# lqhl/rabitq-rs

Hardware: AMD Instinct MI355X
Metric: queries/sec at recall@10>=0.95, GIST-1M d=960, batch=1024 (higher is better)
Workload: dtype u8

## Files before the change

rabitq-rs_amd/csrc/device/k_query.hip:

```cpp
#include <hip/hip_runtime.h>

#include <algorithm>
#include <cstdlib>

#include "launch.hpp"
#include "query_kernels.hpp"
#include "rank_mfma.hpp"
#include "latency.hpp"

namespace rbq {

namespace {
uint32_t next_pow2(uint32_t x) { uint32_t p = 1; while (p < x) p <<= 1; return p; }
}

hipError_t launch_prep(const PrepParams& p, int device, hipStream_t s) {
    if (p.rotator == 0  || p.wg_prep) {
        static LdsAttrCache attr;
        const size_t lds = (size_t)p.D * 4 * 2;
        if (probe_stage(0, reinterpret_cast<const void*>(&k_prep), dim3(p.nq), kThreads, lds)) return hipSuccess;
        hipError_t e = attr.ensure(reinterpret_cast<const void*>(&k_prep), lds, device);
        if (e != hipSuccess) return e;
        hipLaunchKernelGGL(k_prep, dim3(p.nq), dim3(kThreads), lds, s, p.queries, p.dim, p.D, p.Dc, p.rotator, p.rot_blob, p.trunc,
                           p.fac, p.ex_bits, p.rot, p.lut, p.consts, p.rot_hi, p.rot_lo);
// ... 76 lines not shown
    const uint32_t np2 = next_pow2(p.nprobe);
    const size_t lds = (key_window ? 0 : (size_t)np2 * 8) + (size_t)p.D * 4 + kThreads * 4;
    static LdsAttrCache attr, attr_unf;
    const bool unf = p.numeric_variant == (uint32_t)kVarPortable;
    const void* fn = unf ? reinterpret_cast<const void*>(&k_select<true>) : reinterpret_cast<const void*>(&k_select<false>);
    if (probe_stage(2, fn, dim3(p.nq), kThreads, lds)) return hipSuccess;
    hipError_t e = (unf ? attr_unf : attr).ensure(fn, lds, device);
    if (e != hipSuccess) return e;
    if (unf) hipLaunchKernelGGL(k_select<true>, dim3(p.nq), dim3(kThreads), lds, s, (const float*)p.scores, p.nlist, p.nprobe, np2, p.metric, p.rot,
                                p.cent, p.D, p.list_gb0, p.list_n, p.probe, p.wl, p.wl_stride, p.nstream, p.nvec, p.prof_total, p.consts,
                                p.bsum, key_window);
    else hipLaunchKernelGGL(k_select<false>, dim3(p.nq), dim3(kThreads), lds, s, (const float*)p.scores, p.nlist, p.nprobe, np2, p.metric, p.rot,
                       p.cent, p.D, p.list_gb0, p.list_n, p.probe, p.wl, p.wl_stride, p.nstream, p.nvec, p.prof_total, p.consts,
                       p.bsum, key_window);
    return hipGetLastError();
}

namespace {
template <int RM, int V>
hipError_t launch_select_rmv(const SelectParams& p, const SelectGeom& g, size_t lds, int device, hipStream_t s) {
    static LdsAttrCache attr;
    if (probe_stage(2, reinterpret_cast<const void*>(&k_select_mfma<RM, V>), dim3(p.nq), kThreads, lds)) return hipSuccess;
    hipError_t e = attr.ensure(reinterpret_cast<const void*>(&k_select_mfma<RM, V>), lds, device);
    if (e != hipSuccess) return e;
    hipLaunchKernelGGL((k_select_mfma<RM, V>), dim3(p.nq), dim3(kThreads), lds, s, p, g);
    return hipGetLastError();
}
template <int RM>
hipError_t launch_select_rm(const SelectParams& p, const SelectGeom& g, size_t lds, int device, hipStream_t s) {
    if (p.numeric_variant == (uint32_t)kVarAvx2) return launch_select_rmv<RM, kVarAvx2>(p, g, lds, device, s);
    if (p.numeric_variant == (uint32_t)kVarPortable) return launch_select_rmv<RM, kVarPortable>(p, g, lds, device, s);
    return launch_select_rmv<RM, kVarAvx512>(p, g, lds, device, s);
}
}

template <int RM>
size_t select_static_lds() {
    static const size_t v = [] {
        hipFuncAttributes fa;
        if (hipFuncGetAttributes(&fa, reinterpret_cast<const void*>(&k_select_mfma<RM>)) != hipSuccess) { (void)hipGetLastError(); return (size_t)8192; }
        return (size_t)fa.sharedSizeBytes;
    }();
    return v;
}

hipError_t launch_select_mfma(const SelectParams& p, int device, hipStream_t s) {
    SelectGeom g;
    g.cap2 = next_pow2(2 * p.nprobe) < 64u ? 64u : next_pow2(2 * p.nprobe);
    const size_t lds0 = (size_t)g.cap2 * 8 + (size_t)p.D * 4 + kThreads * 4;
    g.row_in_lds = (p.nlist > 4096 && (size_t)p.nlist * 4 <= 65536 &&
                    lds0 + (size_t)p.nlist * 4 + select_static_lds<1>() <= kLdsPerWorkgroupMax) ? 1 : 0;
    size_t lds = lds0 + (g.row_in_lds ? (size_t)p.nlist * 4 : 0);
    g.stage = lds + (size_t)p.nprobe * 16 <= 48 * 1024 ? 1 : 0;
    if (g.stage) lds += (size_t)p.nprobe * 16;
#ifndef RBQ_SEL_ROWS
#define RBQ_SEL_ROWS 4
#endif
    const size_t rowsN = RBQ_SEL_ROWS * ((size_t)p.D + 8) * 4 + 16;
    g.stage_rows = (p.lazy && lds + rowsN <= 64 * 1024) ? (uint32_t)RBQ_SEL_ROWS : 0u;
    g.hx_nv = 0;
    size_t regionN = g.stage_rows ? rowsN : 0;
    if (p.lazy && p.head_exact && p.lut && p.top_k <= kHxMaxVec && p.D % 16 == 0) {
#ifndef RBQ_HX_BUDGET
#define RBQ_HX_BUDGET (16384u * 8u)
#endif
        uint32_t nv = (uint32_t)(((uint32_t)RBQ_HX_BUDGET / p.Dc) / 32u * 32u);
        nv = nv < 64u ? 64u : (nv > kHxMaxVec ? kHxMaxVec : nv);
        const size_t hxN = (hx_scratch_bytes(p.D, p.Dc, p.ex_bits, nv) + 15) & ~(size_t)15;
        if (lds + std::max(regionN, hxN) <= 64 * 1024) { g.hx_nv = nv; regionN = std::max(regionN, hxN); }
    }
    lds += regionN;
    g.cand_cap = (uint32_t)(((g.stage ? (size_t)p.nprobe * 16 : 0) + (g.stage_rows ? rowsN - 16 : 0)) / 8);
    if (p.nlist <= 4096) return launch_select_rm<2>(p, g, lds, device, s);
    if (g.row_in_lds) return launch_select_rm<1>(p, g, lds, device, s);
    return launch_select_rm<0>(p, g, lds, device, s);
}

hipError_t launch_probes_given(const ProbesGivenParams& p, hipStream_t s) {
    if (p.numeric_variant == (uint32_t)kVarPortable)
        hipLaunchKernelGGL(k_probes_given<true>, dim3(p.nq), dim3(kThreads), (size_t)p.D * 4 + kThreads * 4, s, p.list_ids, p.list_counts,
                           p.max_lists, p.nlist, p.metric, p.rot, p.cent, p.D, p.list_gb0, p.list_n, p.probe, p.wl, p.wl_stride, p.nstream,
                           p.consts, p.bsum);
    else hipLaunchKernelGGL(k_probes_given<false>, dim3(p.nq), dim3(kThreads), (size_t)p.D * 4 + kThreads * 4, s, p.list_ids, p.list_counts,
                            p.max_lists, p.nlist, p.metric, p.rot, p.cent, p.D, p.list_gb0, p.list_n, p.probe, p.wl, p.wl_stride, p.nstream,
                            p.consts, p.bsum);
    return hipGetLastError();
}

}
```

rabitq-rs_amd/csrc/device/rank_mfma.hpp:

```cpp
#pragma once
#include "kernels.hpp"

namespace rbq {

#ifndef RBQ_CANON_UNROLL
#define RBQ_CANON_UNROLL 4
#endif
typedef float f32x16 __attribute__((ext_vector_type(16)));

template <int METRIC, int TW>
__global__ __launch_bounds__(256) void k_rank_mfma(const float* __restrict__ rot, const float* __restrict__ cent,
                                                   const QueryConsts* __restrict__ consts,
                                                   const float* __restrict__ cnorm2, uint32_t nq, uint32_t nlist,
                                                   uint32_t D, float* __restrict__ scores) {
    constexpr int BM = 64 * TW, BN = 64 * TW, BK = 32, LD = BK + 1;
    __shared__ float As[BM][LD];
    __shared__ float Bs[BN][LD];
    const uint32_t tid = threadIdx.x, lane = tid & 63u, w = tid >> 6, wm = w >> 1, wn = w & 1u;
    const uint32_t q0 = blockIdx.y * BM, c0 = blockIdx.x * BN;
    f32x16 acc[TW][TW];
#pragma unroll
    for (int a = 0; a < TW; ++a)
#pragma unroll
        for (int b = 0; b < TW; ++b)
// ... 237 lines not shown
    }
    for (uint32_t i = Dmain; i < D; ++i) {
        float p;
        if (METRIC == 0) {
            const float d = qrot[i] - c[i];
            p = d * d;
        } else {
            p = qrot[i] * c[i];
        }
        sum = sum + p;
    }
    return sum;
}

__device__ __forceinline__ void canon_pair2_ip_l2(const float* qrot, const float* __restrict__ c, uint32_t D, uint32_t h,
                                                  float& dot, float& l2) {
    const uint32_t Dmain = D & ~7u;
    float a[4] = {0, 0, 0, 0}, b[4] = {0, 0, 0, 0};
#pragma unroll 4
    for (uint32_t i = 4 * h; i < Dmain; i += 8) {
        const float4 cv = *reinterpret_cast<const float4*>(c + i);
        const float4 qv = *reinterpret_cast<const float4*>(qrot + i);
        const float q4[4] = {qv.x, qv.y, qv.z, qv.w}, c4[4] = {cv.x, cv.y, cv.z, cv.w};
#pragma unroll
        for (int k = 0; k < 4; ++k) {
            const float p = q4[k] * c4[k];
            const float d = q4[k] - c4[k];
            const float r = d * d;
            a[k] = a[k] + p;
            b[k] = b[k] + r;
        }
    }
    float s0 = 0.0f, s1 = 0.0f;
    if (Dmain) {
        s0 = -0.0f; s1 = -0.0f;
#pragma unroll
        for (int l = 0; l < 2; ++l)
#pragma unroll
            for (int k = 0; k < 4; ++k) {
                s0 = s0 + __shfl(a[k], l, 2);
                s1 = s1 + __shfl(b[k], l, 2);
            }
    }
    for (uint32_t i = Dmain; i < D; ++i) {
        const float p = qrot[i] * c[i];
        const float d = qrot[i] - c[i];
        const float r = d * d;
        s0 = s0 + p;
        s1 = s1 + r;
    }
    dot = s0; l2 = s1;
}

#ifdef RBQ_SEL_WAVES
#define RBQ_SEL_BOUNDS __launch_bounds__(kThreads, RBQ_SEL_WAVES)
#else
#define RBQ_SEL_BOUNDS __launch_bounds__(kThreads)
#endif

struct SelectGeom {
    uint32_t cap2;
    int row_in_lds;
    int stage;
    uint32_t stage_rows;
    uint32_t cand_cap;
    uint32_t hx_nv;
};
#ifndef RBQ_HX_TRIGGER
#define RBQ_HX_TRIGGER 6
#endif
#ifndef RBQ_HX_REFINE_MULT
#define RBQ_HX_REFINE_MULT 2
#endif
constexpr uint32_t kHxTrigger = RBQ_HX_TRIGGER;
constexpr uint32_t kHxMaxVec = 256;

template <typename IdxFn>
__device__ __forceinline__ void canon_score_pairs(uint64_t* keys, const float* qrot, const float* __restrict__ cent, uint32_t D, int metric,
                                                  float* grow, uint32_t m, uint32_t tid, IdxFn idx_of) {
    const uint32_t l2 = tid & 1u, grp = tid >> 1;
    for (uint32_t i0 = 0; i0 < m; i0 += kThreads / 2) {
        const uint32_t j = i0 + grp;
        uint32_t cid = 0, e = 0;
        float s = 0.0f;
        if (j < m) {
            e = idx_of(j);
            cid = (uint32_t)keys[e];
            const float* c = cent + (size_t)cid * D;
            if (metric == 0) s = canon_pair2<0>(qrot, c, D, l2);
            else {
                float dl2;
                canon_pair2_ip_l2(qrot, c, D, l2, s, dl2);
                if (l2 == 0) grow[cid] = dl2;
            }
        }
        if (j < m && l2 == 0) keys[e] = make_key(s, cid, metric);
    }
}
template <typename IdxFn>
__device__ __forceinline__ void canon_score_staged(uint64_t* keys, const float* qrot, const float* __restrict__ cent, uint32_t D, int metric,
                                                   float* grow, uint32_t m, uint32_t tid, float* rows, uint32_t RB, IdxFn idx_of) {
    const uint32_t Dp = D + 8u, Dmain = D & ~7u, nv4 = D >> 2;
    for (uint32_t base = 0; base < m; base += RB) {
        const uint32_t nr = m - base < RB ? m - base : RB;
        for (uint32_t x0 = tid; x0 < nr * nv4; x0 += 4 * kThreads) {
            float4 t4[4];
#pragma unroll
            for (int u = 0; u < 4; ++u) {
                const uint32_t x = x0 + (uint32_t)u * kThreads;
                t4[u] = make_float4(0.0f, 0.0f, 0.0f, 0.0f);
                if (x < nr * nv4) {
                    const uint32_t r = x / nv4, j4 = x - r * nv4;
                    const uint32_t cid = (uint32_t)keys[idx_of(base + r)];
                    t4[u] = *reinterpret_cast<const float4*>(cent + (size_t)cid * D + 4 * j4);
                }
            }
#pragma unroll
            for (int u = 0; u < 4; ++u) {
                const uint32_t x = x0 + (uint32_t)u * kThreads;
                if (x < nr * nv4) {
                    const uint32_t r = x / nv4, j4 = x - r * nv4;
                    *reinterpret_cast<float4*>(rows + (size_t)r * Dp + 4 * j4) = t4[u];
                }
            }
        }
// ... 134 lines not shown
        }
    }
}

__device__ __forceinline__ void sort_keys(uint64_t* keys, uint32_t n, uint32_t cap2, uint32_t tid) {
    if (n <= 2 * kThreads) {
        uint64_t my[2] = {~0ull, ~0ull};
        uint32_t rk[2] = {0, 0};
#pragma unroll
        for (int u = 0; u < 2; ++u) if (tid + u * kThreads < n) my[u] = keys[tid + u * kThreads];
        const uint32_t wbase = tid & ~63u;
        if (n > (uint32_t)kThreads) {
#pragma unroll 8
            for (uint32_t j = 0; j < n; ++j) {
                const uint64_t kj = keys[j];
                rk[0] += kj < my[0] ? 1u : 0u;
                rk[1] += kj < my[1] ? 1u : 0u;
            }
        } else if (wbase < n) {
            const uint4* k2 = reinterpret_cast<const uint4*>(keys);
            const uint32_t np2 = (n + 1) >> 1;
#pragma unroll 8
            for (uint32_t j = 0; j < np2; ++j) {
                const uint4 kk = k2[j];
                const uint64_t ka = ((uint64_t)kk.y << 32) | kk.x, kb = ((uint64_t)kk.w << 32) | kk.z;
                rk[0] += (ka < my[0] ? 1u : 0u) + (kb < my[0] ? 1u : 0u);
            }
        }
        __syncthreads();
#pragma unroll
        for (int u = 0; u < 2; ++u) if (tid + u * kThreads < n) keys[rk[u]] = my[u];
        __syncthreads();
    } else {
        for (uint32_t k = 2; k <= cap2; k <<= 1)
            for (uint32_t j = k >> 1; j > 0; j >>= 1) {
                for (uint32_t i = tid; i < cap2; i += kThreads) {
                    const uint32_t ixj = i ^ j;
                    if (ixj > i) {
                        const uint64_t a = keys[i], b = keys[ixj];
                        const bool up = (i & k) == 0;
                        if ((a > b) == up) { keys[i] = b; keys[ixj] = a; }
                    }
                }
                __syncthreads();
            }
    }
}


#ifndef RBQ_HX_EX_ALL
#define RBQ_HX_EX_ALL 0
#endif
#ifndef RBQ_HX_GRANULES
#define RBQ_HX_GRANULES 4
#endif
__host__ __device__ inline size_t hx_scratch_bytes(uint32_t D, uint32_t Dc, uint32_t ex_bits, uint32_t nv) {
    return (size_t)Dc * 4 + (ex_bits ? (size_t)ex_qlen(D, ex_bits) * 4 : 0) + (size_t)nv * 16 + 16;
}
__device__ __forceinline__ uint32_t hx_look8(uint32_t x, const uint8_t* p) {
    uint32_t s = p[x & 15u];
    s += p[16 + ((x >> 4) & 15u)];
    s += p[32 + ((x >> 8) & 15u)];
    s += p[48 + ((x >> 12) & 15u)];
    s += p[64 + ((x >> 16) & 15u)];
    s += p[80 + ((x >> 20) & 15u)];
    s += p[96 + ((x >> 24) & 15u)];
    s += p[112 + (x >> 28)];
    return s;
}
__device__ __forceinline__ bool hx_tame(float x) { return fabsf(x) < 1e30f; }
template <int V, class CostOf>
__device__ __forceinline__ float head_exact_bound(const SelectParams& P, const SelectGeom& G, const QueryConsts& qc, const uint64_t* keys,
                                                  const uint32_t* s_head, const uint32_t* s_hgb, const uint32_t* s_hn, const float* s_hcn,
                                                  uint32_t h, float eps, unsigned char* scratch, const float* qrot, uint32_t* part, uint32_t* hist,
                                                  uint32_t q, uint32_t tid, CostOf&& cost_of) {
    const uint32_t D = P.D, Dc = P.Dc, ex_bits = P.ex_bits, top_k = P.top_k;
    uint32_t r0 = 0, kbest = 0xffffffffu;
    for (uint32_t r = 0; r < h; ++r) {
        const uint32_t k32 = (uint32_t)(keys[s_head[r]] >> 32);
        if (k32 < kbest) { kbest = k32; r0 = r; }
    }
    const float ci = cost_of(kbest);
    const float g_add = ci + 1.01f * eps;
    float ge_lo, ge_hi;
    if (P.metric == 0) { ge_lo = sqrtf(fmaxf(ci - 1.01f * eps, 0.0f)); ge_hi = sqrtf(fmaxf(g_add, 0.0f)); }
    else { const float da = qc.qnorm2 + s_hcn[r0] + 2.0f * ci; ge_lo = sqrtf(fmaxf(da - 4.0f * eps, 0.0f)); ge_hi = sqrtf(fmaxf(da + 4.0f * eps, 0.0f)); }
    const uint32_t gb = s_hgb[r0], nvec = s_hn[r0];
    const uint32_t nv = nvec < G.hx_nv ? nvec : G.hx_nv;
    if (nv < top_k || top_k == 0 || !hx_tame(g_add) || !hx_tame(ge_hi)) return INFINITY;
    if (r0 >= h || (uint64_t)gb + ((nv + 31u) >> 5) > (uint64_t)P.n_blocks) {
        if (tid == 0 && P.fallback_count) atomicAdd(P.fallback_count + 2, 1u);
        return INFINITY;
    }
    if (tid == 0 && P.fallback_count) atomicAdd(P.fallback_count + 3, 1u);
    uint8_t* lutL = scratch;
    float* sq = reinterpret_cast<float*>(scratch + (size_t)Dc * 4);
    const uint32_t qlen = ex_bits ? ex_qlen(D, ex_bits) : 0u;
    float* vEst = sq + qlen;
    float* vLb = vEst + nv;
    float* vIp = vLb + nv;
    float* vU = vIp + nv;
    {
        const uint4* src = reinterpret_cast<const uint4*>(P.lut + (size_t)q * Dc * 4);
        uint4* dst = reinterpret_cast<uint4*>(lutL);
        for (uint32_t i = tid; i < Dc / 4; i += kThreads) dst[i] = src[i];
        for (uint32_t i = tid; i < qlen; i += kThreads) sq[i] = i < D ? qrot[i] : 0.0f;
    }
// ... 96 lines not shown
                const float d = a + m;
                const bool ok = vEst[v] < INFINITY && hx_tame(fa) && hx_tame(fr) && hx_tame(t0) && hx_tame(sacc) && hx_tame(t1) && hx_tame(tt2) &&
                                hx_tame(a) && hx_tame(m) && hx_tame(d);
                vU[j] = ok ? fmaxf(d, vLb[v]) : INFINITY;
            }
        }
    }
    __syncthreads();
    if (tid < R) {
        const float my = vU[tid];
        uint32_t rk = 0;
        for (uint32_t j = 0; j < R; ++j) { const float o = vU[j]; rk += (o < my || (o == my && j < tid)) ? 1u : 0u; }
        if (rk == top_k - 1u) res[0] = my;
    }
    __syncthreads();
    const float r = res[0];
    __syncthreads();
    return r;
}

constexpr uint32_t kSelHead = 4;
constexpr uint32_t kSelTodoMax = 512;
constexpr uint32_t kSelKeptMax = 256;
constexpr uint32_t kSelZoneMax = 1024;

template <int RM, int V = kVarAvx512>
__global__ RBQ_SEL_BOUNDS void k_select_mfma(const SelectParams P, const SelectGeom G) {
    extern __shared__ __align__(16) unsigned char smraw[];
    const uint32_t nlist = P.nlist, nprobe = P.nprobe, cap2 = G.cap2, D = P.D;
    const int metric = P.metric;
    uint64_t* keys = reinterpret_cast<uint64_t*>(smraw);
    float* qrot = reinterpret_cast<float*>(smraw + (size_t)cap2 * 8);
    uint32_t* part = reinterpret_cast<uint32_t*>(qrot + D);
    __shared__ uint32_t hist[256];
    __shared__ uint32_t s_k, s_cnt, s_bad;
    __shared__ unsigned long long s_nvec;
#ifdef RBQ_SEL_STAMPS
    unsigned long long ts[8]; int tn = 0;
#define SSTAMP() ts[tn++] = __builtin_amdgcn_s_memtime()
#else
#define SSTAMP()
#endif
#if defined(RBQ_SEL_STAMPS) && RBQ_SEL_STAMPS == 4
    unsigned long long ls[8] = {0, 0, 0, 0, 0, 0, 0, 0};
#define LSTAMP(i) ls[i] = __builtin_amdgcn_s_memtime()
#else
#define LSTAMP(i)
#endif
    SSTAMP();
    const uint32_t q = blockIdx.x, tid = threadIdx.x;
    float* grow = P.scores + (size_t)q * nlist;
    float* lrow = reinterpret_cast<float*>(part + kThreads);
    uint32_t* pgeo = reinterpret_cast<uint32_t*>(lrow + (RM == 1 ? nlist : 0u));
    float* rows = reinterpret_cast<float*>(smraw + ((reinterpret_cast<unsigned char*>(pgeo + (G.stage ? 4u * nprobe : 0u)) - smraw + 15) & ~(size_t)15));
    constexpr int KPT = 16;
    uint32_t kreg[KPT];
    bool bad_load = false;
    uint64_t* cand = reinterpret_cast<uint64_t*>(pgeo);
    bool use_cand = false;
    uint32_t n_cand = 0;
    auto okey = [&](float s) -> uint32_t {
        int32_t k = total_key(s);
        if (metric == 1) k = ~k;
        return (uint32_t)k ^ 0x80000000u;
    };
    auto cost_of = [&](uint32_t k32) -> float {
        int32_t k = (int32_t)(k32 ^ 0x80000000u);
        if (metric == 1) k = ~k;
        const float s = key_to_float(k);
        return metric == 0 ? s : -s;
    };
    if (RM == 2) {
#pragma unroll
        for (int v = 0; v < KPT / 4; ++v) {
            const uint32_t i = v * 1024u + tid * 4u;
            float4 x = make_float4(0, 0, 0, 0);
            if (i + 3 < nlist) x = *reinterpret_cast<const float4*>(grow + i);
            else { if (i < nlist) x.x = grow[i]; if (i + 1 < nlist) x.y = grow[i + 1]; if (i + 2 < nlist) x.z = grow[i + 2]; }
            bad_load |= !finite_f(x.x) || !finite_f(x.y) || !finite_f(x.z) || !finite_f(x.w);
            kreg[4 * v] = okey(x.x); kreg[4 * v + 1] = okey(x.y); kreg[4 * v + 2] = okey(x.z); kreg[4 * v + 3] = okey(x.w);
        }
    } else if (RM == 1) {
        for (uint32_t i = tid; i < nlist; i += kThreads) lrow[i] = grow[i];
    }
    auto each_key = [&](auto&& body) {
        if (RM == 2) {
#pragma unroll
            for (int u = 0; u < KPT; ++u) {
                const uint32_t i = (uint32_t)(u >> 2) * 1024u + tid * 4u + (uint32_t)(u & 3);
                if (i < nlist) body(i, kreg[u]);
            }
        } else if (RM == 1) {
            for (uint32_t i = tid; i < nlist; i += kThreads) { const float v = lrow[i]; bad_load |= !finite_f(v); body(i, okey(v)); }
        } else if (use_cand) {
            for (uint32_t j = tid; j < n_cand; j += kThreads) { const uint64_t kc = cand[j]; body((uint32_t)kc, (uint32_t)(kc >> 32)); }
        } else {
            for (uint32_t i = tid; i < nlist; i += kThreads) { const float v = grow[i]; bad_load |= !finite_f(v); body(i, okey(v)); }
        }
    };

    {
        float qv[4];
        for (uint32_t i0 = tid; i0 < D; i0 += 4 * kThreads) {
#pragma unroll
            for (int u = 0; u < 4; ++u) qv[u] = i0 + (uint32_t)u * kThreads < D ? P.rot[(size_t)q * D + i0 + (uint32_t)u * kThreads] : 0.0f;
#pragma unroll
            for (int u = 0; u < 4; ++u) if (i0 + (uint32_t)u * kThreads < D) qrot[i0 + (uint32_t)u * kThreads] = qv[u];
        }
    }
    if (tid == 0) { s_k = nprobe - 1; s_cnt = 0; s_nvec = 0; s_bad = 0; }
    __syncthreads();

    SSTAMP();
    bool all = nprobe >= nlist;
    __shared__ uint32_t s_lo, s_hi, s_bin, s_cum, s_h, s_ng, s_w4[4], s_nc;
    auto kth_key = [&](auto&& each, uint32_t k) -> uint32_t {
        if (tid == 0) { s_lo = 0xffffffffu; s_hi = 0u; s_ng = 0u; }
        __syncthreads();
        {
            uint32_t kmn = 0xffffffffu, kmx = 0u;
            each([&](uint32_t, uint32_t key) {
                kmn = key < kmn ? key : kmn;
                kmx = key > kmx ? key : kmx;
            });
            const bool bad = bad_load;
            kmn = wave_min_u32(kmn);
            kmx = ~wave_min_u32(~kmx);
            if ((tid & 63u) == 0) { atomicMin(&s_lo, kmn); atomicMax(&s_hi, kmx); }
            if (bad) s_bad = 1;
        }
        __syncthreads();
        uint32_t lo = s_lo, hi = s_hi;
        while (true) {
            const uint32_t span = hi - lo;
            const uint32_t sh = span < 256u ? 0u : (32u - (uint32_t)__builtin_clz(span)) - 8u;
            hist[tid] = 0;
            __syncthreads();
            each([&](uint32_t, uint32_t key) {
                if (key - lo <= hi - lo) atomicAdd(&hist[(key - lo) >> sh], 1u);
            });
            __syncthreads();
            const uint32_t h = hist[tid];
            uint32_t total;
            const uint32_t excl = block_scan_excl256(h, s_w4, tid, total);
            if (excl <= k && k < excl + h) { s_bin = tid; s_cum = excl; s_h = h; }
            __syncthreads();
            k -= s_cum;
            lo += s_bin << sh;
            const uint32_t width = (sh ? (1u << sh) : 1u) - 1u;
            if (hi - lo > width) hi = lo + width;
            if (sh == 0) break;
            const uint32_t nc = s_h;
            if (nc <= (uint32_t)kThreads) {
                uint32_t* cnd = hist;
                each([&](uint32_t, uint32_t key) {
                    if (key - lo <= hi - lo) cnd[atomicAdd(&s_ng, 1u)] = key;
                });
                __syncthreads();
                if (tid < nc) {
                    const uint32_t my = cnd[tid];
                    uint32_t less = 0, eq = 0;
#pragma unroll 8
                    for (uint32_t j = 0; j < nc; ++j) {
                        const uint32_t kj = cnd[j];
                        less += kj < my ? 1u : 0u;
                        eq += kj == my ? 1u : 0u;
                    }
                    if (less <= k && k < less + eq) s_lo = my;
                }
                __syncthreads();
                lo = s_lo;
                break;
            }
        }
        __syncthreads();
        return lo;
    };
    const QueryConsts qc = P.consts[q];
    const float eps = ((6.0f * (float)D + 16.0f) * 5.9604645e-8f + 4.0f * 1.52587890625e-5f) * (qc.qnorm2 + P.cnorm2_max) * 1.001f;
    auto widen = [&](uint32_t key) -> uint32_t {
        int32_t k = (int32_t)(key ^ 0x80000000u);
        if (metric == 1) k = ~k;
        const float sc = key_to_float(k);
        const float lim = metric == 0 ? sc + 2.0f * eps : sc - 2.0f * eps;
        return finite_f(lim) ? okey(lim) : 0xffffffffu;
    };
    constexpr int KL = 8;
    if (RM == 0 && !all && G.cand_cap >= 4u * nprobe && 2u * nprobe <= (uint32_t)(kThreads * KL)) {
        uint32_t lk[KL];
#pragma unroll
        for (int u = 0; u < KL; ++u) lk[u] = 0xffffffffu;
        constexpr int KU = 8;
        for (uint32_t i0 = tid; i0 < nlist; i0 += kThreads * KU) {
            float vv[KU];
#pragma unroll
            for (int w = 0; w < KU; ++w) { const uint32_t i = i0 + (uint32_t)w * kThreads; vv[w] = i < nlist ? grow[i] : 0.0f; }
#pragma unroll
            for (int w = 0; w < KU; ++w) {
                if (i0 + (uint32_t)w * kThreads < nlist) {
                    const float v = vv[w];
                    bad_load |= !finite_f(v);
                    const uint32_t key = okey(v);
                    if (key < lk[KL - 1]) {
                        lk[KL - 1] = key;
#pragma unroll
                        for (int u = KL - 1; u > 0; --u) {
                            const uint32_t a = lk[u - 1], b = lk[u];
                            lk[u - 1] = a < b ? a : b;
                            lk[u] = a < b ? b : a;
                        }
                    }
                }
            }
        }
        const uint32_t B = kth_key([&](auto&& body) {
#pragma unroll
            for (int u = 0; u < KL; ++u) if (lk[u] != 0xffffffffu) body(0u, lk[u]);
        }, nprobe - 1);
        const uint32_t cutB = widen(B);
        if (tid == 0) s_nc = 0;
        __syncthreads();
        if (cutB != 0xffffffffu && s_bad == 0) {
            for (uint32_t i0 = tid; i0 < nlist; i0 += kThreads * KU) {
                float vv[KU];
#pragma unroll
                for (int w = 0; w < KU; ++w) { const uint32_t i = i0 + (uint32_t)w * kThreads; vv[w] = i < nlist ? grow[i] : 0.0f; }
#pragma unroll
                for (int w = 0; w < KU; ++w) {
                    const uint32_t i = i0 + (uint32_t)w * kThreads;
                    const uint32_t key = okey(vv[w]);
                    if (i < nlist && key <= cutB) {
                        const uint32_t pp = atomicAdd(&s_nc, 1u);
                        if (pp < G.cand_cap) cand[pp] = ((uint64_t)key << 32) | i;
                    }
                }
            }
            __syncthreads();
            n_cand = s_nc;
            use_cand = n_cand <= G.cand_cap && n_cand >= nprobe;
        }
        __syncthreads();
    }
    uint32_t tau_key = 0;
    if (!all) tau_key = kth_key(each_key, nprobe - 1);
    else {
        each_key([&](uint32_t, uint32_t) {});
        if (bad_load) s_bad = 1;
        __syncthreads();
    }
    SSTAMP();
    const uint32_t cut = all ? 0xffffffffu : widen(tau_key);
    __shared__ uint32_t s_cntle, s_minab;
    for (uint32_t i = tid; i < cap2; i += kThreads) keys[i] = ~0ull;
    __shared__ uint32_t s_z0, s_tub, s_flag, s_need, s_dead, s_maxh, s_nh, s_nk, s_head[kSelHead];
    __shared__ unsigned long long s_memvec;
    if (tid == 0) { s_cntle = 0; s_minab = 0xffffffffu;
                    s_z0 = 0; s_tub = (uint32_t)total_key(INFINITY); s_flag = 0; s_need = 0; s_dead = 0; s_maxh = (uint32_t)total_key(-INFINITY); s_memvec = 0; s_nh = 0; s_nk = 0; }
    if (tid < kSelHead) s_head[tid] = 0xffffffffu;
    __syncthreads();
    bool fallback = s_bad != 0 || P.force_fallback != 0;
    if (!fallback) {
        uint32_t cle = 0, mab = 0xffffffffu;
        each_key([&](uint32_t i, uint32_t key) {
            if (key <= cut) {
                const uint32_t p = atomicAdd(&s_cnt, 1u);
                if (p < cap2) keys[p] = ((uint64_t)key << 32) | i;
                if (all || key <= tau_key) ++cle;
                else mab = key < mab ? key : mab;
            }
        });
        cle = wave_sum_u32(cle);
        mab = wave_min_u32(mab);
        if ((tid & 63u) == 0) { if (cle) atomicAdd(&s_cntle, cle); if (mab != 0xffffffffu) atomicMin(&s_minab, mab); }
        __syncthreads();
        fallback = s_cnt > cap2 || s_cnt < nprobe;
    }
    __syncthreads();
    SSTAMP();
    const uint32_t l2 = tid & 1u, grp = tid >> 1;
    uint32_t m_scan = nprobe;
    uint32_t dbg_tub = 0x7fc00000u, dbg_z = 0;
    uint32_t dead_vec = 0;
    if (!fallback) {
        const uint32_t n = s_cnt;
        LSTAMP(0);
        __shared__ uint32_t s_wmin[4][kSelHead], s_todo[kSelTodoMax];
        const uint32_t nown = (n + kThreads - 1 - tid) / kThreads;
        unsigned long long m_certain = 0ull, m_dead = 0ull, m_apx = 0ull;
        BlockSummary ls_own = {0.0f, 0.0f, 0.0f, 0.0f, 0.0f, 0.0f, 0u, 0u};
        uint32_t gb_own = 0, n_own = 0;
        float cn_own = 0.0f;
        if (P.lazy && tid < n) {
            const uint32_t cid = (uint32_t)keys[tid];
            ls_own = P.lsum[cid]; gb_own = P.list_gb0[cid]; n_own = P.list_n[cid];
            if (metric == 1) cn_own = P.cnorm2[cid];
        }
        const uint32_t bound_key = (!all && s_cntle > nprobe) ? tau_key : s_minab;
        const float cost_bound = (all || bound_key == 0xffffffffu) ? INFINITY : cost_of(bound_key);
        {
            uint32_t cnt = 0;
            for (uint32_t u = 0; u < nown && tid < n; ++u) {
                const uint32_t k32 = (uint32_t)(keys[tid + u * kThreads] >> 32);
                if (all || k32 <= tau_key) m_apx |= 1ull << u;
                const bool cert = cost_of(k32) + 2.01f * eps < cost_bound;
                if (cert) { m_certain |= 1ull << u; ++cnt; }
            }
            cnt = wave_sum_u32(cnt);
            if ((tid & 63u) == 0 && cnt) atomicAdd(&s_z0, cnt);
        }
        {
            uint32_t prev = 0;
            const uint32_t wave = tid >> 6;
#pragma unroll
            for (uint32_t r = 0; r < kSelHead; ++r) {
                uint32_t best = 0xffffffffu;
                for (uint32_t u = 0; u < nown && tid < n; ++u) {
                    const uint32_t k32 = (uint32_t)(keys[tid + u * kThreads] >> 32);
                    if ((r == 0 || k32 > prev) && k32 < best) best = k32;
                }
                best = wave_min_u32(best);
                if ((tid & 63u) == 0) s_wmin[wave][r] = best;
                prev = best;
            }
        }
        __syncthreads();
        const uint32_t z0 = s_z0;
#ifdef RBQ_PREP_STAMPS
        const bool lazy_ok = false;
#else
        const bool lazy_ok = P.lazy != 0 && z0 > 0 && n - z0 <= kSelZoneMax && qc.amax <= 65535.0f && P.top_k > 0;
#endif
        uint32_t h = 0;
        if (lazy_ok) {
            uint32_t prev = 0, lvl = 0xffffffffu;
#pragma unroll
            for (uint32_t r = 0; r < kSelHead; ++r) {
                uint32_t best = 0xffffffffu;
#pragma unroll
                for (int w = 0; w < 4; ++w)
#pragma unroll
                    for (uint32_t j = 0; j < kSelHead; ++j) {
                        const uint32_t v = s_wmin[w][j];
                        if ((r == 0 || v > prev) && v < best) best = v;
                    }
                if (best != 0xffffffffu) lvl = best;
                prev = best;
            }
            for (uint32_t u = 0; u < nown && tid < n; ++u) {
                const uint32_t i = tid + u * kThreads;
                if (((m_certain >> u) & 1ull) && (uint32_t)(keys[i] >> 32) <= lvl) {
                    const uint32_t p = atomicAdd(&s_nh, 1u);
                    if (p < kSelHead) s_head[p] = i;
                }
            }
            __syncthreads();
            h = s_nh < kSelHead ? s_nh : kSelHead;
        }
        const uint32_t hp0 = lazy_ok ? s_head[0] : 0xffffffffu, hp1 = lazy_ok ? s_head[1] : 0xffffffffu,
                       hp2 = lazy_ok ? s_head[2] : 0xffffffffu, hp3 = lazy_ok ? s_head[3] : 0xffffffffu;
        auto is_head = [&](uint32_t i) { return i == hp0 || i == hp1 || i == hp2 || i == hp3; };
        bool lazy = false;
        LSTAMP(1);
        if (lazy_ok && h > 0) {
            __shared__ uint32_t s_hgb[kSelHead], s_hn[kSelHead];
            __shared__ float s_hcn[kSelHead];
            if (tid < kSelHead) { s_hgb[tid] = 0; s_hn[tid] = 0; s_hcn[tid] = 0.0f; }
            if (tid == 0) s_need = h;
            __syncthreads();
#pragma unroll
            for (uint32_t r = 0; r < kSelHead; ++r) {
                const uint32_t pos = r == 0 ? hp0 : r == 1 ? hp1 : r == 2 ? hp2 : hp3;
                if (r < h && (pos & (kThreads - 1)) == tid) {
                    uint32_t gb = gb_own, nv = n_own;
                    float cn = cn_own;
                    if (pos >= (uint32_t)kThreads) { const uint32_t cid = (uint32_t)keys[pos]; gb = P.list_gb0[cid]; nv = P.list_n[cid]; if (metric == 1) cn = P.cnorm2[cid]; }
                    s_hgb[r] = gb; s_hn[r] = nv; s_hcn[r] = cn;
                }
            }
            __syncthreads();
            LSTAMP(2);
            auto head_info = [&](uint32_t r, float& g_add, float& g_err, uint32_t& gb, uint32_t& nvec) {
                const uint64_t key = keys[s_head[r]];
                const float ci = cost_of((uint32_t)(key >> 32));
                g_add = ci + 1.01f * eps;
                if (metric == 0) g_err = sqrtf(fmaxf(g_add, 0.0f));
                else g_err = sqrtf(fmaxf(qc.qnorm2 + s_hcn[r] + 2.0f * ci + 4.0f * eps, 0.0f));
                gb = s_hgb[r]; nvec = s_hn[r];
            };
            const uint32_t nb0 = (s_hn[0] + 31u) >> 5, nb1 = (s_hn[1] + 31u) >> 5, nb2 = (s_hn[2] + 31u) >> 5, nb3 = (s_hn[3] + 31u) >> 5;
            static_assert(kSelHead == 4, "four head lists");
            const uint32_t tot = nb0 + nb1 + nb2 + nb3;
            const uint32_t ncand = tot < (uint32_t)kThreads ? tot : (uint32_t)kThreads;
            float myU = INFINITY;
            uint32_t myN = 0;
            if (tid < ncand) {
                uint32_t r = 0, b = tid;
                if (b >= nb0) { b -= nb0; r = 1; if (b >= nb1) { b -= nb1; r = 2; if (b >= nb2) { b -= nb2; r = 3; } } }
                float g_add, g_err; uint32_t gb, nvec;
                head_info(r, g_add, g_err, gb, nvec);
                const BlockSummary bs = P.bsum[gb + b];
                const BlockSummaryEx bx = P.bsumx[gb + b];
                myU = block_ub(bs, bx, g_add, g_err, qc, D, P.ex_bits, P.slack, V == kVarPortable) + 1e-4f * eps;
                myN = (b + 1 == ((nvec + 31u) >> 5)) ? nvec - b * 32u : 32u;
                if (P.head_ub) {
                    uint32_t* hu = P.head_ub + (size_t)q * kHeadUbRow + 10 + 3 * tid;
                    hu[0] = gb + b; hu[1] = __float_as_uint(myU); hu[2] = myN;
                }
            }
            float* candU = reinterpret_cast<float*>(part);
            candU[tid] = myU; hist[tid] = myN;
            if (tid < h) {
                float g_add, g_err; uint32_t gb, nvec;
                head_info(tid, g_add, g_err, gb, nvec);
                if (P.head_ub) {
                    uint32_t* hu = P.head_ub + (size_t)q * kHeadUbRow;
                    hu[2 + 2 * tid] = __float_as_uint(g_add); hu[3 + 2 * tid] = __float_as_uint(g_err);
                    if (tid == 0) { hu[0] = ncand; hu[1] = h; }
                }
                atomicMax(reinterpret_cast<int*>(&s_maxh), total_key(g_add));
            }
            __syncthreads();
            if (tid < ncand && myU < INFINITY) {
                uint32_t cum = 0;
#pragma unroll 8
                for (uint32_t j = 0; j < ncand; ++j) cum += candU[j] <= myU ? hist[j] : 0u;
                if (cum >= P.top_k) atomicMin(reinterpret_cast<int*>(&s_tub), total_key(myU));
            }
            __syncthreads();
            float T_ub = P.fault_dead_all ? -INFINITY : key_to_float((int32_t)s_tub);
            const float cost_maxh = key_to_float((int32_t)s_maxh);
            bool hx_done = false;
            if (P.filter) {
                T_ub = (G.hx_nv && P.head_exact) ? head_exact_bound<V>(P, G, qc, keys, s_head, s_hgb, s_hn, s_hcn, h, eps, reinterpret_cast<unsigned char*>(rows), qrot, part, hist, q, tid, cost_of) : INFINITY;
                hx_done = true;
                if (P.fault_dead_all) T_ub = -INFINITY;
            }
            lazy = T_ub < INFINITY;
            dbg_tub = __float_as_uint(T_ub);
            if (tid < h) s_todo[tid] = s_head[tid];
            LSTAMP(3);
            if (lazy) {
                auto classify = [&](float T) {
                    for (uint32_t u = 0; u < nown && tid < n; ++u) {
                        const uint32_t i = tid + u * kThreads;
                        if (is_head(i)) continue;
                        const uint64_t key = keys[i];
                        const uint32_t cid = (uint32_t)key;
                        const float ci = cost_of((uint32_t)(key >> 32));
                        const float clo = ci - 1.01f * eps, chi = ci + 1.01f * eps;
                        float ge_lo, ge_hi;
                        if (metric == 0) { ge_lo = sqrtf(fmaxf(clo, 0.0f)); ge_hi = sqrtf(fmaxf(chi, 0.0f)); }
                        else {
                            const float da = qc.qnorm2 + (u == 0 ? cn_own : P.cnorm2[cid]) + 2.0f * ci;
                            ge_lo = sqrtf(fmaxf(da - 4.0f * eps, 0.0f)); ge_hi = sqrtf(fmaxf(da + 4.0f * eps, 0.0f));
                        }
                        const BlockSummary ls = u == 0 ? ls_own : P.lsum[cid];
                        const bool dead = clo > cost_maxh && list_bound_reaches(ls, clo, chi, ge_lo, ge_hi, qc, T, V == kVarPortable);
                        if (dead) m_dead |= 1ull << u;
                        else {
                            if (!((m_certain >> u) & 1ull)) s_flag = 1u;
                            const uint32_t p = atomicAdd(&s_need, 1u);
                            if (p < kSelTodoMax) s_todo[p] = i;
                        }
                    }
                    __syncthreads();
                };
                classify(T_ub);
                const uint32_t need1 = s_need;
                __syncthreads();
                if (G.hx_nv && P.head_exact && !hx_done && need1 - h > kHxTrigger) {
                    const float T2 = head_exact_bound<V>(P, G, qc, keys, s_head, s_hgb, s_hn, s_hcn, h, eps, reinterpret_cast<unsigned char*>(rows), qrot, part, hist, q, tid, cost_of);
                    if (T2 < T_ub) {
                        m_dead = 0ull;
                        if (tid == 0) { s_need = h; s_flag = 0u; }
                        __syncthreads();
                        classify(T2);
                        dbg_tub = __float_as_uint(T2);
                    }
                }
                const bool zone_scored = s_flag != 0u || P.exact_members != 0;
                if (zone_scored) {
                    for (uint32_t u = 0; u < nown && tid < n; ++u) {
                        const uint32_t i = tid + u * kThreads;
                        if (!is_head(i) && ((m_dead >> u) & 1ull) && !((m_certain >> u) & 1ull)) {
                            const uint32_t p = atomicAdd(&s_need, 1u);
                            if (p < kSelTodoMax) s_todo[p] = i;
                        }
                    }
                    __syncthreads();
                }
                LSTAMP(4);
                lazy = s_need <= kSelTodoMax;
                dbg_z = (z0 & 0x3ffu) | ((n & 0x3ffu) << 10) | (((s_need - h) & 0xfffu) << 20);
                if (lazy) {
                    const uint32_t m = s_need;
                    if (m) {
                        auto todo_idx = [&](uint32_t j) { return s_todo[j]; };
                        if (G.stage_rows && m <= 2u * G.stage_rows) canon_score_staged(keys, qrot, P.cent, D, metric, grow, m, tid, rows, G.stage_rows, todo_idx);
                        else {
                            if (m <= 64u) canon_score_octets(keys, qrot, P.cent, D, metric, grow, m, tid, todo_idx);
                            else canon_score_pairs(keys, qrot, P.cent, D, metric, grow, m, tid, todo_idx);
                            __threadfence_block();
                            __syncthreads();
                        }
                    }
                    LSTAMP(5);
                    __shared__ uint32_t s_zone[512];
                    __shared__ unsigned long long s_kept[kSelKeptMax];
                    if (zone_scored) {
                        for (uint32_t w = tid; w < 512; w += kThreads) s_zone[w] = 0u;
                        __syncthreads();
                        for (uint32_t u = 0; u < nown && tid < n; ++u)
                            if (!((m_certain >> u) & 1ull)) { const uint32_t i = tid + u * kThreads; atomicOr(&s_zone[i >> 5], 1u << (i & 31u)); }
                        __syncthreads();
                    }
                    unsigned long long m_keep = 0ull;
                    uint32_t dv = 0;
                    unsigned long long mv = 0;
                    for (uint32_t u = 0; u < nown && tid < n; ++u) {
                        const uint32_t i = tid + u * kThreads;
                        const bool cert = (m_certain >> u) & 1ull, dead = (m_dead >> u) & 1ull;
                        bool member = cert;
                        if (!cert && zone_scored) {
                            const uint64_t my = keys[i];
                            uint32_t less = 0;
                            for (uint32_t j = 0; j < n; ++j) less += ((s_zone[j >> 5] >> (j & 31u)) & 1u) && keys[j] < my ? 1u : 0u;
                            member = less < nprobe - z0;
                        }
                        if (dead && P.audit_dead) {
                            uint32_t* ad = P.audit_dead + (size_t)q * (kAuditCap + 1);
                            const uint32_t pa = atomicAdd(ad, 1u);
                            if (pa < kAuditCap) ad[1 + pa] = (uint32_t)keys[i];
                        }
                        if (member && !dead) {
                            m_keep |= 1ull << u;
                            const uint32_t p = atomicAdd(&s_nk, 1u);
                            if (p < kSelKeptMax) s_kept[p] = keys[i];
                        }
                        if (P.exact_members ? member : (P.prof_total != nullptr && ((m_apx >> u) & 1ull))) {
                            const uint32_t nvec = P.list_n[(uint32_t)keys[i]];
                            mv += nvec;
                            if (dead && P.exact_members) dv += nvec;
                        }
                    }
                    if (dv) atomicAdd(&s_dead, dv);
                    if (mv) atomicAdd(&s_memvec, mv);
                    __syncthreads();
                    if (s_nk <= kSelKeptMax) {
                        m_scan = s_nk;
                        if (tid < m_scan) {
                            const unsigned long long my = s_kept[tid];
// ... 317 lines not shown
```

Before: 7.611 million.

## Tune select kernel: register-based kth-key, shared pgeo LDS, occupancy bounds

For the small-nlist path the select kernel now tracks per-thread min/max of the register keys and finds the nprobe-th key with a range histogram plus a small candidate rank pass, falling back to the generic routine when needed. It also overlaps the pgeo staging area with the rows/hx region, cuts staged rows and hx granules, and sets default launch bounds to 6 waves. Several shared values are made wave-uniform with readfirstlane, and shortlist init is hoisted before the first barrier to drop one sync. This trims LDS use and barrier count to raise occupancy, at the cost of possible register spills and less staging capacity.

After: 7.228 million. -5.0%, worse.

```diff
diff --git a/rabitq-rs_amd/csrc/device/k_query.hip b/rabitq-rs_amd/csrc/device/k_query.hip
--- a/rabitq-rs_amd/csrc/device/k_query.hip
+++ b/rabitq-rs_amd/csrc/device/k_query.hip
@@ -152,12 +152,18 @@
                     lds0 + (size_t)p.nlist * 4 + select_static_lds<1>() <= kLdsPerWorkgroupMax) ? 1 : 0;
     size_t lds = lds0 + (g.row_in_lds ? (size_t)p.nlist * 4 : 0);
     g.stage = lds + (size_t)p.nprobe * 16 <= 48 * 1024 ? 1 : 0;
-    if (g.stage) lds += (size_t)p.nprobe * 16;
+    g.pgeo_shared = (g.stage && p.nlist <= 4096) ? 1 : 0;
+    const size_t pgeoN = g.stage ? (size_t)p.nprobe * 16 : 0;
+    if (g.stage && !g.pgeo_shared) lds += pgeoN;
 #ifndef RBQ_SEL_ROWS
 #define RBQ_SEL_ROWS 4
 #endif
-    const size_t rowsN = RBQ_SEL_ROWS * ((size_t)p.D + 8) * 4 + 16;
-    g.stage_rows = (p.lazy && lds + rowsN <= 64 * 1024) ? (uint32_t)RBQ_SEL_ROWS : 0u;
+#ifndef RBQ_SEL_ROWS_REG
+#define RBQ_SEL_ROWS_REG 2
+#endif
+    const uint32_t sel_rows = p.nlist <= 4096 ? (uint32_t)RBQ_SEL_ROWS_REG : (uint32_t)RBQ_SEL_ROWS;
+    const size_t rowsN = sel_rows * ((size_t)p.D + 8) * 4 + 16;
+    g.stage_rows = (p.lazy && lds + rowsN <= 64 * 1024) ? sel_rows : 0u;
     g.hx_nv = 0;
     size_t regionN = g.stage_rows ? rowsN : 0;
     if (p.lazy && p.head_exact && p.lut && p.top_k <= kHxMaxVec && p.D % 16 == 0) {
@@ -169,6 +175,7 @@
         const size_t hxN = (hx_scratch_bytes(p.D, p.Dc, p.ex_bits, nv) + 15) & ~(size_t)15;
         if (lds + std::max(regionN, hxN) <= 64 * 1024) { g.hx_nv = nv; regionN = std::max(regionN, hxN); }
     }
+    if (g.pgeo_shared) regionN = std::max(regionN, pgeoN);
     lds += regionN;
     g.cand_cap = (uint32_t)(((g.stage ? (size_t)p.nprobe * 16 : 0) + (g.stage_rows ? rowsN - 16 : 0)) / 8);
     if (p.nlist <= 4096) return launch_select_rm<2>(p, g, lds, device, s);
diff --git a/rabitq-rs_amd/csrc/device/rank_mfma.hpp b/rabitq-rs_amd/csrc/device/rank_mfma.hpp
--- a/rabitq-rs_amd/csrc/device/rank_mfma.hpp
+++ b/rabitq-rs_amd/csrc/device/rank_mfma.hpp
@@ -313,7 +313,10 @@
     dot = s0; l2 = s1;
 }
 
-#ifdef RBQ_SEL_WAVES
+#ifndef RBQ_SEL_WAVES
+#define RBQ_SEL_WAVES 6
+#endif
+#if RBQ_SEL_WAVES > 0
 #define RBQ_SEL_BOUNDS __launch_bounds__(kThreads, RBQ_SEL_WAVES)
 #else
 #define RBQ_SEL_BOUNDS __launch_bounds__(kThreads)
@@ -323,6 +326,7 @@
     uint32_t cap2;
     int row_in_lds;
     int stage;
+    int pgeo_shared;
     uint32_t stage_rows;
     uint32_t cand_cap;
     uint32_t hx_nv;
@@ -332,6 +336,9 @@
 #endif
 #ifndef RBQ_HX_REFINE_MULT
 #define RBQ_HX_REFINE_MULT 2
+#endif
+#ifndef RBQ_SEL_STAGED_ROUNDS
+#define RBQ_SEL_STAGED_ROUNDS 2
 #endif
 constexpr uint32_t kHxTrigger = RBQ_HX_TRIGGER;
 constexpr uint32_t kHxMaxVec = 256;
@@ -572,7 +579,7 @@
 #define RBQ_HX_EX_ALL 0
 #endif
 #ifndef RBQ_HX_GRANULES
-#define RBQ_HX_GRANULES 4
+#define RBQ_HX_GRANULES 2
 #endif
 __host__ __device__ inline size_t hx_scratch_bytes(uint32_t D, uint32_t Dc, uint32_t ex_bits, uint32_t nv) {
     return (size_t)Dc * 4 + (ex_bits ? (size_t)ex_qlen(D, ex_bits) * 4 : 0) + (size_t)nv * 16 + 16;
@@ -775,13 +782,15 @@
     float* grow = P.scores + (size_t)q * nlist;
     float* lrow = reinterpret_cast<float*>(part + kThreads);
     uint32_t* pgeo = reinterpret_cast<uint32_t*>(lrow + (RM == 1 ? nlist : 0u));
-    float* rows = reinterpret_cast<float*>(smraw + ((reinterpret_cast<unsigned char*>(pgeo + (G.stage ? 4u * nprobe : 0u)) - smraw + 15) & ~(size_t)15));
+    float* rows = reinterpret_cast<float*>(smraw + ((reinterpret_cast<unsigned char*>(pgeo + (G.stage && !G.pgeo_shared ? 4u * nprobe : 0u)) - smraw + 15) & ~(size_t)15));
     constexpr int KPT = 16;
     uint32_t kreg[KPT];
+    uint32_t kmn0 = 0xffffffffu, kmx0 = 0u;
     bool bad_load = false;
     uint64_t* cand = reinterpret_cast<uint64_t*>(pgeo);
     bool use_cand = false;
     uint32_t n_cand = 0;
+    auto uni = [](uint32_t x) -> uint32_t { return (uint32_t)__builtin_amdgcn_readfirstlane((int)x); };
     auto okey = [&](float s) -> uint32_t {
         int32_t k = total_key(s);
         if (metric == 1) k = ~k;
@@ -802,6 +811,12 @@
             else { if (i < nlist) x.x = grow[i]; if (i + 1 < nlist) x.y = grow[i + 1]; if (i + 2 < nlist) x.z = grow[i + 2]; }
             bad_load |= !finite_f(x.x) || !finite_f(x.y) || !finite_f(x.z) || !finite_f(x.w);
             kreg[4 * v] = okey(x.x); kreg[4 * v + 1] = okey(x.y); kreg[4 * v + 2] = okey(x.z); kreg[4 * v + 3] = okey(x.w);
+#pragma unroll
+            for (int c = 0; c < 4; ++c)
+                if (i + (uint32_t)c < nlist) {
+                    kmn0 = kreg[4 * v + c] < kmn0 ? kreg[4 * v + c] : kmn0;
+                    kmx0 = kreg[4 * v + c] > kmx0 ? kreg[4 * v + c] : kmx0;
+                }
         }
     } else if (RM == 1) {
         for (uint32_t i = tid; i < nlist; i += kThreads) lrow[i] = grow[i];
@@ -832,11 +847,29 @@
         }
     }
     if (tid == 0) { s_k = nprobe - 1; s_cnt = 0; s_nvec = 0; s_bad = 0; }
+    __shared__ uint32_t s_lo, s_hi, s_bin, s_cum, s_h, s_ng, s_w4[4], s_nc;
+    __shared__ uint32_t s_cntle, s_minab;
+    __shared__ uint32_t s_z0, s_tub, s_flag, s_need, s_dead, s_maxh, s_nh, s_nk, s_head[kSelHead];
+    __shared__ unsigned long long s_memvec;
+    __shared__ uint32_t s_wmn[4], s_wmx[4], s_wbad[4];
+    auto init_shortlist = [&]() {
+        for (uint32_t i = tid; i < cap2; i += kThreads) keys[i] = ~0ull;
+        if (tid == 0) { s_cntle = 0; s_minab = 0xffffffffu;
+                        s_z0 = 0; s_tub = (uint32_t)total_key(INFINITY); s_flag = 0; s_need = 0; s_dead = 0; s_maxh = (uint32_t)total_key(-INFINITY); s_memvec = 0; s_nh = 0; s_nk = 0; }
+        if (tid < kSelHead) s_head[tid] = 0xffffffffu;
+    };
+    if (RM == 2) {
+        const uint32_t wmn = wave_min_u32(kmn0), wmx = ~wave_min_u32(~kmx0);
+        const bool wbad = __builtin_amdgcn_ballot_w64(bad_load) != 0ull;
+        if ((tid & 63u) == 0) { s_wmn[tid >> 6] = wmn; s_wmx[tid >> 6] = wmx; s_wbad[tid >> 6] = wbad ? 1u : 0u; }
+        hist[tid] = 0;
+        if (tid == 0) s_ng = 0u;
+        init_shortlist();
+    }
     __syncthreads();
 
     SSTAMP();
     bool all = nprobe >= nlist;
-    __shared__ uint32_t s_lo, s_hi, s_bin, s_cum, s_h, s_ng, s_w4[4], s_nc;
     auto kth_key = [&](auto&& each, uint32_t k) -> uint32_t {
         if (tid == 0) { s_lo = 0xffffffffu; s_hi = 0u; s_ng = 0u; }
         __syncthreads();
@@ -899,6 +932,45 @@
         __syncthreads();
         return lo;
     };
+    auto kth_key_regs = [&](const uint32_t k0) -> uint32_t {
+        uint32_t k = k0, lo = s_wmn[0], hi = s_wmx[0];
+#pragma unroll
+        for (int w = 1; w < 4; ++w) { lo = s_wmn[w] < lo ? s_wmn[w] : lo; hi = s_wmx[w] > hi ? s_wmx[w] : hi; }
+        const uint32_t span = hi - lo;
+        const uint32_t sh = span < 256u ? 0u : (32u - (uint32_t)__builtin_clz(span)) - 8u;
+        each_key([&](uint32_t, uint32_t key) { atomicAdd(&hist[(key - lo) >> sh], 1u); });
+        __syncthreads();
+        const uint32_t h = hist[tid];
+        uint32_t total;
+        const uint32_t excl = block_scan_excl256(h, s_w4, tid, total);
+        if (excl <= k && k < excl + h) { s_bin = tid; s_cum = excl; s_h = h; }
+        __syncthreads();
+        k -= s_cum;
+        lo += s_bin << sh;
+        const uint32_t width = (sh ? (1u << sh) : 1u) - 1u;
+        if (hi - lo > width) hi = lo + width;
+        if (sh == 0) return lo;
+        const uint32_t nc = s_h;
+        if (nc > (uint32_t)kThreads) return kth_key(each_key, k0);
+        uint32_t* cnd = hist;
+        each_key([&](uint32_t, uint32_t key) {
+            if (key - lo <= hi - lo) cnd[atomicAdd(&s_ng, 1u)] = key;
+        });
+        __syncthreads();
+        if (tid < nc) {
+            const uint32_t my = cnd[tid];
+            uint32_t less = 0, eq = 0;
+#pragma unroll 8
+            for (uint32_t j = 0; j < nc; ++j) {
+                const uint32_t kj = cnd[j];
+                less += kj < my ? 1u : 0u;
+                eq += kj == my ? 1u : 0u;
+            }
+            if (less <= k && k < less + eq) s_lo = my;
+        }
+        __syncthreads();
+        return uni(s_lo);
+    };
     const QueryConsts qc = P.consts[q];
     const float eps = ((6.0f * (float)D + 16.0f) * 5.9604645e-8f + 4.0f * 1.52587890625e-5f) * (qc.qnorm2 + P.cnorm2_max) * 1.001f;
     auto widen = [&](uint32_t key) -> uint32_t {
@@ -965,7 +1037,8 @@
         __syncthreads();
     }
     uint32_t tau_key = 0;
-    if (!all) tau_key = kth_key(each_key, nprobe - 1);
+    if (RM == 2) { if (!all) tau_key = kth_key_regs(nprobe - 1); }
+    else if (!all) tau_key = kth_key(each_key, nprobe - 1);
     else {
         each_key([&](uint32_t, uint32_t) {});
         if (bad_load) s_bad = 1;
@@ -973,15 +1046,11 @@
     }
     SSTAMP();
     const uint32_t cut = all ? 0xffffffffu : widen(tau_key);
-    __shared__ uint32_t s_cntle, s_minab;
-    for (uint32_t i = tid; i < cap2; i += kThreads) keys[i] = ~0ull;
-    __shared__ uint32_t s_z0, s_tub, s_flag, s_need, s_dead, s_maxh, s_nh, s_nk, s_head[kSelHead];
-    __shared__ unsigned long long s_memvec;
-    if (tid == 0) { s_cntle = 0; s_minab = 0xffffffffu;
-                    s_z0 = 0; s_tub = (uint32_t)total_key(INFINITY); s_flag = 0; s_need = 0; s_dead = 0; s_maxh = (uint32_t)total_key(-INFINITY); s_memvec = 0; s_nh = 0; s_nk = 0; }
-    if (tid < kSelHead) s_head[tid] = 0xffffffffu;
-    __syncthreads();
-    bool fallback = s_bad != 0 || P.force_fallback != 0;
+    if (RM != 2) {
+        init_shortlist();
+        __syncthreads();
+    }
+    bool fallback = (RM == 2 ? (s_wbad[0] | s_wbad[1] | s_wbad[2] | s_wbad[3]) != 0u : s_bad != 0) || P.force_fallback != 0;
     if (!fallback) {
         uint32_t cle = 0, mab = 0xffffffffu;
         each_key([&](uint32_t i, uint32_t key) {
@@ -998,14 +1067,14 @@
         __syncthreads();
         fallback = s_cnt > cap2 || s_cnt < nprobe;
     }
-    __syncthreads();
+    if (RM != 2) __syncthreads();
     SSTAMP();
     const uint32_t l2 = tid & 1u, grp = tid >> 1;
     uint32_t m_scan = nprobe;
     uint32_t dbg_tub = 0x7fc00000u, dbg_z = 0;
     uint32_t dead_vec = 0;
     if (!fallback) {
-        const uint32_t n = s_cnt;
+        const uint32_t n = uni(s_cnt);
         LSTAMP(0);
         __shared__ uint32_t s_wmin[4][kSelHead], s_todo[kSelTodoMax];
         const uint32_t nown = (n + kThreads - 1 - tid) / kThreads;
@@ -1047,7 +1116,7 @@
             }
         }
         __syncthreads();
-        const uint32_t z0 = s_z0;
+        const uint32_t z0 = uni(s_z0);
 #ifdef RBQ_PREP_STAMPS
         const bool lazy_ok = false;
 #else
@@ -1077,10 +1146,10 @@
                 }
             }
             __syncthreads();
-            h = s_nh < kSelHead ? s_nh : kSelHead;
-        }
-        const uint32_t hp0 = lazy_ok ? s_head[0] : 0xffffffffu, hp1 = lazy_ok ? s_head[1] : 0xffffffffu,
-                       hp2 = lazy_ok ? s_head[2] : 0xffffffffu, hp3 = lazy_ok ? s_head[3] : 0xffffffffu;
+            h = uni(s_nh < kSelHead ? s_nh : kSelHead);
+        }
+        const uint32_t hp0 = uni(lazy_ok ? s_head[0] : 0xffffffffu), hp1 = uni(lazy_ok ? s_head[1] : 0xffffffffu),
+                       hp2 = uni(lazy_ok ? s_head[2] : 0xffffffffu), hp3 = uni(lazy_ok ? s_head[3] : 0xffffffffu);
         auto is_head = [&](uint32_t i) { return i == hp0 || i == hp1 || i == hp2 || i == hp3; };
         bool lazy = false;
         LSTAMP(1);
@@ -1163,7 +1232,7 @@
             if (tid < h) s_todo[tid] = s_head[tid];
             LSTAMP(3);
             if (lazy) {
-                auto classify = [&](float T) {
+                auto classify = [&](float T, const bool own) {
                     for (uint32_t u = 0; u < nown && tid < n; ++u) {
                         const uint32_t i = tid + u * kThreads;
                         if (is_head(i)) continue;
@@ -1174,10 +1243,10 @@
                         float ge_lo, ge_hi;
                         if (metric == 0) { ge_lo = sqrtf(fmaxf(clo, 0.0f)); ge_hi = sqrtf(fmaxf(chi, 0.0f)); }
                         else {
-                            const float da = qc.qnorm2 + (u == 0 ? cn_own : P.cnorm2[cid]) + 2.0f * ci;
+                            const float da = qc.qnorm2 + (own && u == 0 ? cn_own : P.cnorm2[cid]) + 2.0f * ci;
                             ge_lo = sqrtf(fmaxf(da - 4.0f * eps, 0.0f)); ge_hi = sqrtf(fmaxf(da + 4.0f * eps, 0.0f));
                         }
-                        const BlockSummary ls = u == 0 ? ls_own : P.lsum[cid];
+                        const BlockSummary ls = own && u == 0 ? ls_own : P.lsum[cid];
                         const bool dead = clo > cost_maxh && list_bound_reaches(ls, clo, chi, ge_lo, ge_hi, qc, T, V == kVarPortable);
                         if (dead) m_dead |= 1ull << u;
                         else {
@@ -1188,7 +1257,7 @@
                     }
                     __syncthreads();
                 };
-                classify(T_ub);
+                if (hx_done) classify(T_ub, false); else classify(T_ub, true);
                 const uint32_t need1 = s_need;
                 __syncthreads();
                 if (G.hx_nv && P.head_exact && !hx_done && need1 - h > kHxTrigger) {
@@ -1197,7 +1266,7 @@
                         m_dead = 0ull;
                         if (tid == 0) { s_need = h; s_flag = 0u; }
                         __syncthreads();
-                        classify(T2);
+                        classify(T2, false);
                         dbg_tub = __float_as_uint(T2);
                     }
                 }
@@ -1219,7 +1288,7 @@
                     const uint32_t m = s_need;
                     if (m) {
                         auto todo_idx = [&](uint32_t j) { return s_todo[j]; };
-                        if (G.stage_rows && m <= 2u * G.stage_rows) canon_score_staged(keys, qrot, P.cent, D, metric, grow, m, tid, rows, G.stage_rows, todo_idx);
+                        if (G.stage_rows && m <= (uint32_t)RBQ_SEL_STAGED_ROUNDS * G.stage_rows) canon_score_staged(keys, qrot, P.cent, D, metric, grow, m, tid, rows, G.stage_rows, todo_idx);
                         else {
                             if (m <= 64u) canon_score_octets(keys, qrot, P.cent, D, metric, grow, m, tid, todo_idx);
                             else canon_score_pairs(keys, qrot, P.cent, D, metric, grow, m, tid, todo_idx);
```
